# liaojing/videomorphing

Measured on AMD Instinct MI355X. Metric: Mpixel*iters/s (halfway optimizer, 1080p pair, 6-level pyramid, 500 iters/level), higher is better.
Workload: dtype f32

## Files before the change

### videomorphing_amd/csrc/vm_sweep_kernels.hip

```cpp
#include <algorithm>
#include <type_traits>
#include "vm_morph_common.h"

typedef __attribute__((address_space(1))) const uint32_t vm_g_cu32;
typedef __attribute__((address_space(1))) uint32_t vm_g_u32;
typedef __attribute__((address_space(1))) const unsigned long long vm_g_cu64;
typedef __attribute__((address_space(1))) unsigned long long vm_g_u64;
typedef __attribute__((address_space(1))) const float vm_g_cf32;

__device__ __forceinline__ int mad24(int a, int b, int c) { return __mul24(a, b) + c; }

namespace {

__device__ __forceinline__ int tile_cols(int w) { return (w + VM_PITCH_X - 1) / VM_PITCH_X; }
__device__ __forceinline__ int tile_rows(int h) { return (h + VM_PITCH_Y - 1) / VM_PITCH_Y; }
__device__ __forceinline__ int tile_ox(int t, int gx, int offx) { return (t % gx) * VM_PITCH_X + offx; }
__device__ __forceinline__ int tile_oy(int t, int gx, int offy) { return (t / gx) * VM_PITCH_Y + offy; }
__device__ __forceinline__ int phase_px(int ox, int slot, int pj) { return ox + (slot & 31) * 2 + pj; }
__device__ __forceinline__ int phase_py(int oy, int slot, int pi) { return oy + (slot >> 5) * 2 + pi; }
__device__ __forceinline__ void stage_imp(uint32_t *imp, const uint32_t *tables, int tid, int T) { for (int k = tid; k < 225; k += T) imp[k] = tables[VM_TAB_IMP + k]; }
__device__ __forceinline__ void stage_tps(float *tps, const uint32_t *tables, int tid, int T) { for (int k = tid; k < 625; k += T) tps[k] = __uint_as_float(tables[VM_TAB_TPS + k]); }
__device__ __forceinline__ float cell_count(int qy, int h, int qx, int w) { return (float)(window_count(qy, h) * window_count(qx, w)); }
__device__ __forceinline__ int window_row(int k) { return (k * 13) >> 6; }

struct TileLds {
    float2 mean[VM_NCELL], var[VM_NCELL], tpsb[VM_NCELL];
    float cross[VM_NCELL], value[VM_NCELL];
    float2 d_mean[256], d_var[256], d_step[256];
    float d_cross[256];
    int d_ok[256];
    int list[256];
    int wave_cnt[4];
    uint32_t cbits[8];
    float tps[625];
    uint32_t imp[225];
    uint32_t mask[6][16];
    uint32_t n_eval;
    uint32_t dirty[(VM_NCELL + 31) / 32];
};

struct SplitLds {
    float2 d_mean[256], d_var[256], d_step[256];
    float d_cross[256];
    int d_ok[256];
    int list[256];
    int wave_cnt[4];
    float tps[625];
    uint32_t imp[225];
    uint32_t mask[6][16];
    uint32_t n_eval;
};

struct PixelCtx {
    int px, py;
    int idx;
    float2 v, old_luma;
    float tps_axy, ui_axy;
    float2 tps_b, ui_b;
    float2 tref;
    float tmask;
};

__device__ __forceinline__ float temp_change(const PixelCtx &c, float dx, float dy)
{
    float v_temp = 0.0f;
    v_temp += fabsf(c.v.x + dx - c.tref.x) - fabsf(c.v.x - c.tref.x);
    v_temp += fabsf(c.v.y + dy - c.tref.y) - fabsf(c.v.y - c.tref.y);
    return v_temp;
}

template <bool TEMP>
__device__ __forceinline__ bool temp_on(const VmLevelView &L) { return TEMP && L.temp_mask != nullptr; }
#if VM_EXACT
#define VM_VARIANT_TEMPLATE
constexpr bool TEMP = true;
#else
// ... 647 lines not shown
    fi = __builtin_amdgcn_fmed3f(fi, -1.0f, (float)L.w);
    fj = __builtin_amdgcn_fmed3f(fj, -1.0f, (float)L.h);
    const int i = clamp0(L.w - 1, (int)fi + t.cx), j = clamp0(L.h - 1, (int)fj + t.cy);
    wgt = fmaf(t.wxs, a, t.wxo) * fmaf(t.wys, b, t.wyo);
    return (uint32_t)(t.imgoff + j * L.rs + i) << 2;
}
__device__ __forceinline__ void taps32_issue(const VmLevelView &L, const TapLane &t, const PixelCtx &c, float vx,
                                             float vy, float &texel, float &wgt)
{
    texel = *(vm_g_cf32 *)((const char *)L.img0 + taps32_addr(L, t, c, vx, vy, wgt));
}
struct TexelKeep {
    uint32_t off = 0xFFFFFFFFu;
    float texel = 0.0f;
};
__device__ __forceinline__ void taps32_issue(const VmLevelView &L, const TapLane &t, const PixelCtx &c, float vx,
                                             float vy, TexelKeep &keep, float &texel, float &wgt)
{
    const uint32_t off = taps32_addr(L, t, c, vx, vy, wgt);
    if (off != keep.off) {
        keep.texel = *(vm_g_cf32 *)((const char *)L.img0 + off);
        keep.off = off;
    }
    texel = keep.texel;
}
__device__ __forceinline__ void taps32_finish(const TapLane &t, float texel, float wgt, float &lx, float &ly)
{
    float r = texel * wgt;
    r += dpp_xor1(r);
    r += dpp_xor2(r);
    const float o = dpp_half_mirror(r);
    lx = t.odd ? o : r;
    ly = t.odd ? r : o;
}
template <int K>
__device__ __forceinline__ float ladder_take(float x)
{
    return __int_as_float(__builtin_amdgcn_ds_swizzle(__float_as_int(x), 0x07 | (K << 8)));
}
__device__ __forceinline__ void taps32(const VmLevelView &L, const TapLane &t, const PixelCtx &c, float vx, float vy,
                                       TexelKeep &keep, float &lx, float &ly)
{
    float texel, wgt;
    taps32_issue(L, t, c, vx, vy, keep, texel, wgt);
    taps32_finish(t, texel, wgt, lx, ly);
}
__device__ __forceinline__ void line_lumas(const VmLevelView &L, const TapLane &t, const PixelCtx &c, float gx, float gy,
                                           float tmin, TexelKeep &keep, float2 &luma)
{
    taps32(L, t, c, fmaf(gx, tmin, c.v.x), fmaf(gy, tmin, c.v.y), keep, luma.x, luma.y);
}

template <bool INTERIOR>
__device__ __forceinline__ float change32(const VmKParams &P, const Nb1 &nb, const PixelCtx &c, float lx, float ly)
{
    const float dmx = lx - c.old_luma.x, dmy = ly - c.old_luma.y;
    const float dvx = lx * lx - c.old_luma.x * c.old_luma.x;
    const float dvy = ly * ly - c.old_luma.y * c.old_luma.y;
    const float dcross = lx * ly - c.old_luma.x * c.old_luma.y;
    float acc;
    if (INTERIOR) {
        const float val = ssim_core(window_mean(nb.A, dmx, 0.04f), window_mean(nb.B, dmy, 0.04f), nb.VX + dvx, nb.VY + dvy,
                                    nb.X + dcross, 25.0f, P.ssim_clamp);
        acc = nb.N != 0.0f ? nb.VAL - val : 0.0f;
    } else {
        const bool valid = nb.N != 0.0f;
        const float n = valid ? nb.N : 25.0f;
        const float in = n == 25.0f ? 0.04f : __builtin_amdgcn_rcpf(n);
        const float val = ssim_core(window_mean(nb.A, dmx, in), window_mean(nb.B, dmy, in), nb.VX + dvx, nb.VY + dvy,
                                    nb.X + dcross, n, P.ssim_clamp);
        acc = valid ? nb.VAL - val : 0.0f;
    }
    return group_sum(acc, 32);
}

template <class Ring>
__device__ __forceinline__ float fover32(const VmLevelView &L, const Ring &ring, const PixelCtx &c, float gx, float gy,
                                         int sub)
{
    const int k = sub & 7, k1 = (k + 1) & 7;
    const float sgn = (sub & 8) ? 1.0f : -1.0f;
    const float vx = sgn * c.v.x, vy = sgn * c.v.y;
    float ex[2], ey[2];
#pragma unroll
    for (int e = 0; e < 2; ++e) {
        const int kk = e ? k1 : k;
        const int rx = ((0x06A4 >> (2 * kk)) & 3) - 1, ry = ((0x6A40 >> (2 * kk)) & 3) - 1;
        const int qx = c.px + rx, qy = c.py + ry;
        float ux = vx, uy = vy;
        const bool in = qx >= 0 && qx < L.w && qy >= 0 && qy < L.h;
        const float2 nv = ring(kk, in ? qy * L.rs + qx : c.idx);
        if (in) {
            ux = sgn * nv.x;
            uy = sgn * nv.y;
        }
        ex[e] = ux + (float)(c.px - rx);
        ey[e] = uy + (float)(c.py - ry);
    }
    float t_min = 10;
    fover_isec((float)c.px + vx, (float)c.py + vy, sgn * gx, sgn * gy, ex[0], ey[0], ex[1], ey[1], t_min);
    return group_min32(sub < 16 ? t_min : 10.0f);
}

template <bool INTERIOR, bool TEMP, class Ring>
__device__ __forceinline__ bool decide32(const VmLevelView &L, const VmKParams &P, const Nb1 &nb, const Ring &ring,
                                         const PixelCtx &c, int sub, float2 &step, float2 &luma,
                                         uint32_t &n_eval)
{
    n_eval += 4;
    const bool has_temp = temp_on<TEMP>(L);
    const float WT = has_temp ? P.w_temp * c.tmask * L.factor_d * L.inv_wh : 0.0f;
    const TapLane tl = tap_lane_make(L, sub);
    float lx, ly;
    float gx = 0, gy = 0;
    float g_tex[4], g_wgt[4];
#pragma unroll
    for (int k = 0; k < 4; ++k) {
        const float sgn = (k & 1) ? -1.0f : 1.0f;
        const float dx = k < 2 ? sgn * P.eps : 0.0f, dy = k < 2 ? 0.0f : sgn * P.eps;
        taps32_issue(L, tl, c, c.v.x + dx, c.v.y + dy, g_tex[k], g_wgt[k]);
    }
#pragma unroll
    for (int k = 0; k < 4; ++k) {
        const float sgn = (k & 1) ? -1.0f : 1.0f;
        const float dx = k < 2 ? sgn * P.eps : 0.0f, dy = k < 2 ? 0.0f : sgn * P.eps;
        taps32_finish(tl, g_tex[k], g_wgt[k], lx, ly);
// ... 38 lines not shown
    float b = cc * C, x = b * R + cc * C;
    float fb, fx;
    ELINE(b, fb);
    ELINE(x, fx);
#pragma unroll 1
    for (;;) {
        if (!(cc - a > P.eps))
            break;
        const bool lt = fx < fb;
        const float p = lt ? x : b, qv = lt ? cc : a;
        a = lt ? b : a;
        cc = lt ? cc : x;
        const float xn = p * R + qv * C;
        float f;
        ELINE(xn, f);
        const float ob = b, ofb = fb;
        b = lt ? x : xn;
        x = lt ? xn : ob;
        fb = lt ? fx : f;
        fx = lt ? f : ofb;
    }
#undef ELINE
    const float tmin = fx < fb ? x : b, fmin = fx < fb ? fx : fb;
    if (!(fmin < 0))
        return false;
    step = make_float2(gx * tmin, gy * tmin);
    line_lumas(L, tl, c, gx, gy, tmin, keep, luma);
    return true;
}


__device__ __forceinline__ float ladder_pick(bool hi, int oct, float l0, float h0, float l1, float h1, float l2, float h2,
                                             float l3, float h3)
{
    const float p0 = hi ? h0 : l0, p1 = hi ? h1 : l1, p2 = hi ? h2 : l2, p3 = hi ? h3 : l3;
    const float p01 = (oct & 1) ? p1 : p0, p23 = (oct & 1) ? p3 : p2;
    return (oct & 2) ? p23 : p01;
}
#define LADDER_FETCH(K_, BLX_, BLY_, PLX_, PLY_, LX_, LY_)  \
    {                                                       \
        if ((K_) == 0) {                                    \
            (LX_) = ladder_take<0>(BLX_);                   \
            (LY_) = ladder_take<0>(BLY_);                   \
        } else {                                            \
            (LX_) = (PLX_);                                 \
            (LY_) = (PLY_);                                 \
        }                                                   \
        if ((K_) != 3) {                                    \
            (PLX_) = ladder_take<((K_) + 1) & 3>(BLX_);     \
            (PLY_) = ladder_take<((K_) + 1) & 3>(BLY_);     \
        }                                                   \
    }
#define GOLDEN64_NO_TRACE(T_)
#define GOLDEN64_NO_BATCH(T_)
#define GOLDEN64_REGIME_ROUND(EVALB_, TRACE_, K_, CC_, EPS_, HI_, NEVAL_)                                              \
    {                                                                                                                  \
        const float xn = b * R, xn2 = xn * R;                                                                          \
        float f1, f2;                                                                                                  \
        EVALB_(K_, (HI_) ? xn2 : xn, f1, f2);                                                                          \
        TRACE_(xn)                                                                                                     \
              \
        const bool held = x > (EPS_) && !(fb < f1);                                                                    \
        if (held) {                           \
            TRACE_(xn2)                                                                                                \
        }                                                                                                              \
        (NEVAL_) += held ? 2 : 1;                                                                                      \
        (CC_) = held ? b : x;                                                                                          \
        x = held ? xn : b;                                                                                             \
        b = held ? xn2 : xn;                                                                                           \
        fx = held ? f1 : fb;                                                                                           \
        fb = held ? f2 : f1;                                                                                           \
    }
#define GOLDEN64(EVAL2_, BATCH_, EVALB_, TRACE_, CC_, EPS_, HI_, OCT_, NEVAL_, TMIN_, FMIN_)                           \
    {                                                                                                                  \
        const float R = 0.618033989f, C = 1.0f - R;                                                                    \
        float a = 0;                                                                                                   \
        float b = (CC_) * C, x = b * R + (CC_) * C;                                                                    \
        float fb, fx;                                                                                                  \
        {                     \
            const float q1 = b * R, q2 = q1 * R, q3 = q2 * R, q4 = q3 * R, q5 = q4 * R, q6 = q5 * R;                   \
            BATCH_(ladder_pick((HI_), (OCT_), b, x, q1, q2, q3, q4, q5, q6))                                           \
        }                                                                                                              \
        EVALB_(0, (HI_) ? x : b, fb, fx);                                                                              \
        TRACE_(b)                                                                                                      \
        TRACE_(x)                                                                                                      \
        (NEVAL_) += 2;                                                                                                 \
        _Pragma("unroll 1") for (;;) {                                          \
            if (!((CC_) > (EPS_) && !(fx < fb)))                                                                       \
                break;                                                                                                 \
            GOLDEN64_REGIME_ROUND(EVALB_, TRACE_, 1, CC_, EPS_, HI_, NEVAL_)                                           \
            if (!((CC_) > (EPS_) && !(fx < fb)))                                                                       \
                break;                                                                                                 \
            GOLDEN64_REGIME_ROUND(EVALB_, TRACE_, 2, CC_, EPS_, HI_, NEVAL_)                                           \
            if (!((CC_) > (EPS_) && !(fx < fb)))                                                                       \
                break;                                                                                                 \
            GOLDEN64_REGIME_ROUND(EVALB_, TRACE_, 3, CC_, EPS_, HI_, NEVAL_)                                           \
            if (!((CC_) > (EPS_) && !(fx < fb)))                                                                       \
                break;                                                                                                 \
            {                       \
                const float q1 = b * R, q2 = q1 * R, q3 = q2 * R, q4 = q3 * R, q5 = q4 * R, q6 = q5 * R, q7 = q6 * R,  \
                            q8 = q7 * R;                                                                               \
                BATCH_(ladder_pick((HI_), (OCT_), q1, q2, q3, q4, q5, q6, q7, q8))                                     \
            }                                                                                                          \
            GOLDEN64_REGIME_ROUND(EVALB_, TRACE_, 0, CC_, EPS_, HI_, NEVAL_)                                           \
        }                                                                                                              \
        _Pragma("unroll 1") for (;;)                                                                                   \
        {                                                                                                              \
            if (!((CC_) - a > (EPS_)))                                                                                 \
                break;                                                                                                 \
            const bool lt = fx < fb;                                                                                   \
                          \
            const float p = lt ? x : b, qv = lt ? (CC_) : a;                                                           \
            const float a1 = lt ? b : a, cc1 = lt ? (CC_) : x;                                                         \
            const float xn = p * R + qv * C;                                                                           \
            const float b1 = lt ? x : xn, x1 = lt ? xn : b;                                                            \
             \
               \
                      \
                                                                               \
            const bool G = lt;                                                                                         \
            const float p2 = G ? x1 : b1, q2 = G ? cc1 : a1;                                                           \
            const float xn2 = p2 * R + q2 * C;                                                                         \
            float f1, f2;                                                                                              \
            EVAL2_((HI_) ? xn2 : xn, f1, f2);                                                                          \
            TRACE_(xn)                                                                                                 \
            ++(NEVAL_);                                                                                                \
            {                                                                                                          \
                const float nfb = lt ? fx : f1, nfx = lt ? f1 : fb;                                                    \
                a = a1;                                                                                                \
                (CC_) = cc1;                                                                                           \
                b = b1;                                                                                                \
                x = x1;                                                                                                \
                fb = nfb;                                                                                              \
                fx = nfx;                                                                                              \
            }                                                                                                          \
            if ((CC_) - a > (EPS_) && (fx < fb) == G) {          \
                TRACE_(xn2)                                                                                            \
                const float ob = b, ofb = fb;                                                                          \
                a = G ? b : a;                                                                                         \
                (CC_) = G ? (CC_) : x;                                                                                 \
                b = G ? x : xn2;                                                                                       \
                x = G ? xn2 : ob;                                                                                      \
                fb = G ? fx : f2;                                                                                      \
                fx = G ? f2 : ofb;                                                                                     \
                ++(NEVAL_);                                                                                            \
            }                                                                                                          \
        }                                                                                                              \
        (TMIN_) = fx < fb ? x : b;                                                                                     \
        (FMIN_) = fx < fb ? fx : fb;                                                                                   \
    }

template <bool INTERIOR, bool LADDER, bool TEMP, class Ring>
__device__ __forceinline__ bool decide64(const VmLevelView &L, const VmKParams &P, const Nb1 &nb, const Ring &ring,
                                         const PixelCtx &c, int sub, bool hi, float2 &step, float2 &luma,
                                         uint32_t &n_eval)
{
    n_eval += 4;
    const bool has_temp = temp_on<TEMP>(L);
    const float WT = has_temp ? P.w_temp * c.tmask * L.factor_d * L.inv_wh : 0.0f;
    const TapLane tl = tap_lane_make(L, sub);
    float lx, ly;
    float gx = 0, gy = 0;
    {
        const float sgn = hi ? -1.0f : 1.0f;
        float g_tex[2], g_wgt[2];
#pragma unroll
        for (int r = 0; r < 2; ++r) {
            const float dx = r == 0 ? sgn * P.eps : 0.0f, dy = r == 0 ? 0.0f : sgn * P.eps;
            taps32_issue(L, tl, c, c.v.x + dx, c.v.y + dy, g_tex[r], g_wgt[r]);
        }
#pragma unroll
        for (int r = 0; r < 2; ++r) {
            const float dx = r == 0 ? sgn * P.eps : 0.0f, dy = r == 0 ? 0.0f : sgn * P.eps;
            taps32_finish(tl, g_tex[r], g_wgt[r], lx, ly);
            const float change = change32<INTERIOR>(P, nb, c, lx, ly);
            const float dd = dx * dx + dy * dy;
            const float v_tps = fmaf(c.tps_axy, dd, fmaf(c.tps_b.x, dx, c.tps_b.y * dy));
            const float v_ui = fmaf(c.ui_axy, dd, fmaf(c.ui_b.x, dx, c.ui_b.y * dy));
            float e = (P.w_ui * v_ui + P.w_ssim * change) * L.inv_wh + P.w_tps * v_tps;
            if (has_temp)
                e = fmaf(WT, temp_change(c, dx, dy), e);
            e *= sgn;
            float e_lo, e_hi;
            halves(e, e_lo, e_hi);
            if (r == 0) {
                gx += e_lo;
                gx += e_hi;
            } else {
                gy += e_lo;
                gy += e_hi;
            }
        }
    }
    gx = -gx;
    gy = -gy;
    const float ng = fsqrt(gx * gx + gy * gy);
    if (ng == 0)
        return false;
    gx = fdiv(gx, ng);
    gy = fdiv(gy, ng);
    float cc = fmaxf(fover32(L, ring, c, gx, gy, sub) - P.eps, 0.0f);
    const float gg = gx * gx + gy * gy;
    const float WS = P.w_ssim * L.inv_wh, WU = P.w_ui * L.inv_wh;
    const float Q2 = (WU * c.ui_axy + P.w_tps * c.tps_axy) * gg;
    const float Q1 = WU * (c.ui_b.x * gx + c.ui_b.y * gy) + P.w_tps * (c.tps_b.x * gx + c.tps_b.y * gy);
    const float T0 = fabsf(c.v.x - c.tref.x) + fabsf(c.v.y - c.tref.y);
    TexelKeep keep;
#define ELINE2(T_, FLO_, FHI_)                                                         \
    {                                                                                  \
        const float nvx_ = fmaf(gx, (T_), c.v.x), nvy_ = fmaf(gy, (T_), c.v.y);        \
        taps32(L, tl, c, nvx_, nvy_, keep, lx, ly);                                    \
        float f_ = fmaf(WS, change32<INTERIOR>(P, nb, c, lx, ly), (T_) * fmaf(Q2, (T_), Q1)); \
        if (has_temp)                                                                  \
            f_ = fmaf(WT, (fabsf(nvx_ - c.tref.x) + fabsf(nvy_ - c.tref.y)) - T0, f_); \
        halves(f_, (FLO_), (FHI_));                                                    \
    }
    float blx, bly;
    float plx, ply;
#define LADDER2(T_)                                                                             \
    if (LADDER)                                                                                 \
        taps32(L, tl, c, fmaf(gx, (T_), c.v.x), fmaf(gy, (T_), c.v.y), keep, blx, bly);
#define ELINE2B(K_, T_, FLO_, FHI_)                                                    \
    {                                                                                  \
        const float nvx_ = fmaf(gx, (T_), c.v.x), nvy_ = fmaf(gy, (T_), c.v.y);        \
        if (LADDER)                                                                    \
            LADDER_FETCH(K_, blx, bly, plx, ply, lx, ly)                               \
        else                                                                           \
            taps32(L, tl, c, nvx_, nvy_, keep, lx, ly);                                \
        float f_ = fmaf(WS, change32<INTERIOR>(P, nb, c, lx, ly), (T_) * fmaf(Q2, (T_), Q1)); \
        if (has_temp)                                                                  \
            f_ = fmaf(WT, (fabsf(nvx_ - c.tref.x) + fabsf(nvy_ - c.tref.y)) - T0, f_); \
        halves(f_, (FLO_), (FHI_));                                                    \
    }
    float tmin, fmin;
    GOLDEN64(ELINE2, LADDER2, ELINE2B, GOLDEN64_NO_TRACE, cc, P.eps, hi, sub >> 3, n_eval, tmin, fmin)
#undef ELINE2
#undef ELINE2B
#undef LADDER2
    if (!(fmin < 0))
        return false;
    step = make_float2(gx * tmin, gy * tmin);
    line_lumas(L, tl, c, gx, gy, tmin, keep, luma);
    return true;
}
#endif

template <bool TEMP = true>
__device__ __forceinline__ void ctx_load(PixelCtx &c, const VmLevelView &L, const float *s_tps, int px, int py)
{
    c.px = px;
    c.py = py;
    c.idx = py * L.rs + px;
    c.v = L.v[c.idx];
    c.old_luma = L.luma[c.idx];
    c.ui_axy = L.ui_axy[c.idx];
    c.ui_b = L.ui_b[c.idx];
    c.tps_axy = s_tps[(border_class(py, L.h) * 5 + border_class(px, L.w)) * 25 + 12] / 2;
    c.tref = make_float2(0, 0);
    c.tmask = 0.0f;
    if (temp_on<TEMP>(L)) {
        c.tref = L.temp_ref[c.idx];
        c.tmask = L.temp_mask[c.idx];
    }
}

__device__ __forceinline__ bool is_interior(const VmLevelView &L, int px, int py)
{
    return px >= 4 && px < L.w - 4 && py >= 4 && py < L.h - 4;
}

struct MaskGeom {
    int bx0, by0, nbx, nby;
};
__device__ __forceinline__ MaskGeom mask_geom(int w, int h, int ox, int oy)
{
    MaskGeom g;
    g.bx0 = ox / 5 - 1;
    g.by0 = oy / 5 - 1;
    const int bx1 = min(ox + VM_TILE_W - 1, w - 1) / 5 + 1;
    const int by1 = min(oy + VM_TILE_H - 1, h - 1) / 5 + 1;
    g.nbx = bx1 - g.bx0 + 1;
    g.nby = by1 - g.by0 + 1;
    return g;
}
__device__ __forceinline__ MaskGeom mask_geom(const VmLevelView &L, int ox, int oy) { return mask_geom(L.w, L.h, ox, oy); }

__device__ __forceinline__ bool mask_hit(const uint32_t (*mask)[16], const uint32_t *imp, const MaskGeom &g,
                                         int px, int py)
{
    const int oxb = px % 5, oyb = py % 5;
// ... 800 lines not shown
        for (int pj = 0; pj < 2; ++pj) {
            const int vx = V.vx, vy = V.vy;
            const int vpi = pi ^ ((oy - vy) & 1), vpj = pj ^ ((ox - vx) & 1);
            int *const ph_cnt = Q.ph_cnt[pj];
            uint32_t *const ph_cand = Q.ph_cand[pj], *const ph_commit = Q.ph_commit[pj];
            bool cand = false, hit = false;
            uint32_t *mword = nullptr;
            uint32_t mbit = 0;
            if (tid < 256) {
                const int px = vx + (tid & 31) * 2 + vpj, py = vy + (tid >> 5) * 2 + vpi;
                if (px >= ox && px <= rx1 && py >= oy && py <= ry1 && mask_hit(S.mask, S.imp, V.g, px, py)) {
                    hit = true;
                    cand = !pixel_locked(L, P.bcond, px, py);
                    mword = &S.mask[py / 5 - V.g.by0][px / 5 - V.g.bx0];
                    mbit = 1u << ((px % 5) + (py % 5) * 5);
                }
                const unsigned long long bc = __ballot(cand), bh = __ballot(hit);
                if ((tid & 63) == 0) {
                    ph_cand[(tid >> 6) * 2] = (uint32_t)bc;
                    ph_cand[(tid >> 6) * 2 + 1] = (uint32_t)(bc >> 32);
                    ph_cnt[tid >> 6] = __popcll(bc) | (bh ? 1 << 16 : 0);
                    ph_commit[(tid >> 6) * 2] = 0;
                    ph_commit[(tid >> 6) * 2 + 1] = 0;
                }
            }
            __syncthreads();
            const int w0 = ph_cnt[0], w1 = ph_cnt[1], w2 = ph_cnt[2], w3 = ph_cnt[3];
            if (!((w0 | w1 | w2 | w3) >> 16))
                continue;
            const int n_act = (w0 & 0xFFFF) + (w1 & 0xFFFF) + (w2 & 0xFFFF) + (w3 & 0xFFFF);
            if (hit && !cand)
                atomicAnd(mword, ~mbit);
            if (n_act > 0) {
                st_cand += n_act;
                const bool wide = n_act * 64 <= T;
                for (int base = 0; base < n_act; base += wide ? T / 64 : T / 32) {
                    const int li = base + (wide ? tid >> 6 : tid >> 5), sub = tid & 31;
                    const bool writer = wide ? (tid & 63) == 0 : sub == 0;
                    const int slot = sv_kth_slot(ph_cand, min(li, n_act - 1));
                    const int tx = slot & 31, ty = slot >> 5;
                    const int px = vx + tx * 2 + vpj, py = vy + ty * 2 + vpi;
                    const bool wave_interior = __all(li >= n_act || is_interior(L, px, py));
                    if (li < n_act) {
                        LdsSrc src{&S, (ty * 2 + vpi) * VM_HALO_W + (tx * 2 + vpj)};
                        const int pc = src.hc + 2 * VM_HALO_W + 2;
                        PixelCtx c;
                        c.px = px;
                        c.py = py;
                        c.idx = py * L.rs + px;
                        c.v = X.v[pc];
                        c.old_luma = X.luma[pc];
                        c.ui_axy = X.uiaxy[pc];
                        c.ui_b = X.uib[pc];
                        c.tps_axy = S.tps[(border_class(py, L.h) * 5 + border_class(px, L.w)) * 25 + 12] / 2;
                        c.tref = make_float2(0, 0);
                        c.tmask = 0.0f;
                        if (temp_on<TEMP>(L)) {
                            c.tref = L.temp_ref[c.idx];
                            c.tmask = L.temp_mask[c.idx];
                        }
                        c.tps_b = S.tpsb[pc];
                        const RingLds ring{X.v, pc};
                        float2 step, luma;
                        Nb1 nb;
                        bool ok;
                        uint32_t n_eval = 0;
                        if (wave_interior) {
                            nb1_load<true>(nb, L, src, c, sub);
                            ok = wide ? decide64<true, true, TEMP>(L, P, nb, ring, c, sub, (tid & 32) != 0, step, luma, n_eval)
                                      : decide32<true, TEMP>(L, P, nb, ring, c, sub, step, luma, n_eval);
                        } else {
                            nb1_load<false>(nb, L, src, c, sub);
                            ok = wide ? decide64<false, true, TEMP>(L, P, nb, ring, c, sub, (tid & 32) != 0, step, luma, n_eval)
                                      : decide32<false, TEMP>(L, P, nb, ring, c, sub, step, luma, n_eval);
                        }
                        if (writer) {
                            atomicAdd(&S.n_eval, n_eval);
                            uint32_t *const mw = &S.mask[py / 5 - V.g.by0][px / 5 - V.g.bx0];
                            const uint32_t mb = 1u << ((px % 5) + (py % 5) * 5);
                            if (ok) {
                                S.d_step[slot] = step;
                                S.d_mean[slot] = commit_dmean(luma, c.old_luma);
                                S.d_var[slot] = commit_dvar(luma, c.old_luma);
                                S.d_cross[slot] = commit_dcross(luma.x, luma.y, c.old_luma.x, c.old_luma.y);
                                X.luma[pc] = luma;
                                X.uib[pc] = commit_ui_b(c.ui_b, c.ui_axy, step);
                                X.v[pc] = commit_v(c.v, step);
                                atomicOr(&X.dirty[pc >> 5], 1u << (pc & 31));
                                atomicOr(&ph_commit[ty], 1u << tx);
                                atomicOr(mw, mb);
                                if (res && (res > 1 || !sv_safe(L, V, px, py)))
                                    Q.unsafe = 1u;
                            } else
                                atomicAnd(mw, ~mb);
                        }
                    }
                }
            }
            __syncthreads();

            uint32_t cb[8];
            int ncommit = 0, ty0 = 8, ty1 = -1;
#pragma unroll
            for (int k = 0; k < 8; ++k) {
                cb[k] = ph_commit[k];
                ncommit += __popc(cb[k]);
                if (cb[k]) {
// ... 662 lines not shown
                                          int qy, float2 &m, float2 &q, float &cr, float2 &tb, int order)
{
#if !VM_EXACT
    (void)order;
#endif
    const bool touched = hits != 0;
#pragma unroll
    for (int half = 0; half < 2; ++half) {
        if (!__any(hits != 0))
            break;
        float4 ra[5], rb[5];
        int bidx[5];
#pragma unroll
        for (int k = 0; k < 5; ++k) {
            if (half == 1 && k == 4) {
                bidx[k] = -1;
                continue;
            }
#if VM_EXACT
            int b = -1;
            if (hits) {
                if (!(order & 2)) {
                    b = (order & 1) ? 31 - __clz(hits) : __ffs(hits) - 1;
                } else {
                    const uint32_t ht = transpose5(hits);
                    const int bt = (order & 1) ? 31 - __clz(ht) : __ffs(ht) - 1;
                    b = (bt % 5) * 5 + bt / 5;
                }
                hits &= ~(1u << b);
            }
#else
            const int b = hits ? __ffs(hits) - 1 : -1;
            hits &= hits - 1;
#endif
            bidx[k] = b;
            const int bb = max(b, 0);
            const int dy = window_row(bb), dx = bb - dy * 5;
            const int rsafe = b >= 0 ? (qy + dy - 2) * L.rs + (qx + dx - 2) : qy * L.rs + qx;
            ra[k] = rec_load<COH>(r_a + rsafe);
            rb[k] = rec_load<COH>(r_b + rsafe);
        }
#pragma unroll
        for (int k = 0; k < 5; ++k) {
            const int b = bidx[k];
            if (b < 0)
                continue;
            const int dy = window_row(b), dx = b - dy * 5;
            const int x = qx + dx - 2, y = qy + dy - 2;
            m.x += ra[k].x;
            m.y += ra[k].y;
            q.x += ra[k].z;
            q.y += ra[k].w;
            cr += rb[k].x;
            const float kk = s_tps[(border_class(y, L.h) * 5 + border_class(x, L.w)) * 25 + (4 - dy) * 5 + (4 - dx)];
            tb.x += rb[k].y * kk;
            tb.y += rb[k].z * kk;
        }
    }
    return touched;
}

template <int T, bool TEMP = true>
__global__ __launch_bounds__(T) __attribute__((amdgpu_waves_per_eu(T / 128))) void SUF(k_step)(const VmLevelView *__restrict__ views, int cap, VmKParams P,
                                                   const uint32_t *__restrict__ tables, int offx, int offy, int pi,
                                                   int pj, int parts, uint32_t epoch, uint32_t pe, int srcbuf,
                                                   int n_fold, uint32_t *__restrict__ flags,
                                                   uint32_t *__restrict__ stats, int iter_idx, int fixed_work,
                                                   uint32_t *__restrict__ slots_cur, const uint32_t *__restrict__ slots_prev,
                                                   int prev_iter_idx, int nslot)
{
    __shared__ StepLds S;
    const int tid = threadIdx.x;
    const VmLevelView L = views[blockIdx.z];
    flags += (size_t)blockIdx.z * cap;
    stats += (size_t)blockIdx.z * cap * VM_STAT_WORDS;
    const bool s1 = srcbuf == 1, d1 = srcbuf == 0;
    const float2 *s_mean = s1 ? L.mean2 : L.mean, *s_var = s1 ? L.var2 : L.var, *s_tpsb = s1 ? L.tps_b2 : L.tps_b;
    const float *s_cross = s1 ? L.cross2 : L.cross, *s_value = s1 ? L.value2 : L.value;
    const uint32_t *s_imp = s1 ? L.impmask2 : L.impmask;
    float2 *d_mean = d1 ? L.mean2 : L.mean, *d_var = d1 ? L.var2 : L.var, *d_tpsb = d1 ? L.tps_b2 : L.tps_b;
    float *d_cross = d1 ? L.cross2 : L.cross, *d_value = d1 ? L.value2 : L.value;
    uint32_t *d_imp = d1 ? L.impmask2 : L.impmask;
    const bool in_place = srcbuf == 2;
    const bool r1 = pe & 1u, w1 = epoch & 1u;
    const uint32_t *r_tag = r1 ? L.rec_tag2 : L.rec_tag;
    const float4 *r_a = r1 ? L.rec_a2 : L.rec_a, *r_b = r1 ? L.rec_b2 : L.rec_b;
    uint32_t *w_tag = w1 ? L.rec_tag2 : L.rec_tag;
    float4 *w_a = w1 ? L.rec_a2 : L.rec_a, *w_b = w1 ? L.rec_b2 : L.rec_b;
    const uint32_t want = (pe << 2) | 1u;

    stage_tps(S.tps, tables, tid, T);
    if (tid < VM_STEP_BH * 4)
        S.bits[tid >> 2][tid & 3] = 0;

    if ((int)blockIdx.x < n_fold) {
        const int nfx = (L.w + 63) / 64;
        const int x0 = ((int)blockIdx.x % nfx) * 64, y0 = ((int)blockIdx.x / nfx) * 16;
        const int bx0 = x0 - 2, by0 = y0 - 2;
        constexpr int NTF = (68 * 20 + T - 1) / T, NCF = 1024 / T;
        uint32_t tg[NTF];
#pragma unroll
        for (int e = 0; e < NTF; ++e) {
            const int k = tid + e * T;
            const int x = bx0 + k % 68, y = by0 + k / 68;
            tg[e] = (k < 68 * 20 && x >= 0 && x < L.w && y >= 0 && y < L.h) ? r_tag[y * L.rs + x] : 0u;
        }
        float2 cm[NCF], cq[NCF], ctb[NCF];
// ... 543 lines not shown
            a_ok[r] = ph > 0 && sub < 25 && x >= ox && x < tx1 && y >= oy && y < ty1;
            a_tag[r] = o_rtag + ((uint32_t)(a_ok[r] ? mad24(y, L.rs, x) : pidx) << 2);
        }
        bool b_ok;
        uint32_t b_tag;
        {
            const int x = 5 * wbx + sub % 5, y = 5 * wby + sub / 5;
            b_ok = ph > 0 && has_word && sub < 25 && x >= ox && x < tx1 && y >= oy && y < ty1;
            b_tag = o_rtag + ((uint32_t)(b_ok ? mad24(y, L.rs, x) : pidx) << 2);
        }
        const int sx0 = -4 + ((ppj ^ pj) & 1), sy0 = -4 + ((ppi ^ pi) & 1);
        bool c_ok;
        uint32_t c_tag, c_rec;
        {
            const int dx = sx0 + 2 * (sub % 5), dy = sy0 + 2 * (sub / 5);
            const int x = px + dx, y = py + dy;
            c_ok = ph > 0 && sub < 25 && dx <= 4 && dy <= 4 && x >= ox && x < tx1 && y >= oy && y < ty1;
            const uint32_t ri = (uint32_t)(c_ok ? mad24(y, L.rs, x) : pidx);
            c_tag = o_rtag + (ri << 2);
            c_rec = (hi ? o_rb : o_ra) + (ri << 4);
        }
        const int phx = 2 + 2 * tx + pj, phy = 2 + 2 * ty + pi;
        const int ohx0 = tx == 0 ? 0 : phx, ohx1 = tx == 31 ? VM_HALO_W - 1 : phx + 1;
        const int ohy0 = ty == 0 ? 0 : phy, ohy1 = ty == 7 ? VM_HALO_H - 1 : phy + 1;
        const int wi_ = window_row(sub), wj_ = sub - wi_ * 5;
        int chx, chy;
        if (sub < 25) {
            chx = phx + wj_ - 2;
            chy = phy + wi_ - 2;
        } else {
            const int xcol = (tx == 0 && pj == 1) ? 0 : ((tx == 31 && pj == 0) ? VM_HALO_W - 1 : -1);
            const int xrow = (ty == 0 && pi == 1) ? 0 : ((ty == 7 && pi == 0) ? VM_HALO_H - 1 : -1);
            const int ncol = xcol >= 0 ? ohy1 - ohy0 + 1 : 0;
            const int e = (sub - 25) + (hi ? 7 : 0);
            chx = chy = -1;
            if (e < ncol) {
                chx = xcol;
                chy = ohy0 + e;
            } else if (xrow >= 0) {
                int k = ohx0 + (e - ncol);
                if (xcol >= 0 && xcol == ohx0)
                    ++k;
                if (k <= ohx1 && k != xcol) {
                    chx = k;
                    chy = xrow;
                }
            }
        }
        const int qx = ox - 2 + chx, qy = oy - 2 + chy;
        const bool cell_ok = chx >= 0 && qx >= 0 && qx < L.w && qy >= 0 && qy < L.h;
        const bool okc = cell_ok && sub < 25;
        const uint32_t gi = (uint32_t)(cell_ok ? mad24(qy, L.rs, qx) : pidx);
        const uint32_t g4 = gi << 2, g8 = gi << 3;
        const float tps_axy = S.tps[(border_class(spy, L.h) * 5 + border_class(spx, L.w)) * 25 + 12] / 2;
        __builtin_amdgcn_sched_barrier(0);
        uint32_t mword[2], mcanon[2], mtag[2];
#pragma unroll
        for (int r = 0; r < 2; ++r) {
            mword[r] = ldo<uint32_t>(sbase, os_imp + a_word[r]);
            mcanon[r] = ldo<uint32_t>(sb, o_imp + a_word[r]);
            mtag[r] = ldo<uint32_t>(wb, a_tag[r]);
        }
        uint32_t otag = ldo<uint32_t>(wb, b_tag);
        uint32_t ctag = ldo<uint32_t>(wb, c_tag);
        const float4 crec = ldo<float4>(wb, c_rec);
        float2 m = ldo<float2>(sbase, os_mean + g8), q = ldo<float2>(sbase, os_var + g8), tb = ldo<float2>(sbase, os_tpsb + g8);
        float cr = ldo<float>(sbase, os_cross + g4), val = ldo<float>(sbase, os_value + g4);
        c.tref = make_float2(0, 0);
        c.tmask = 0.0f;
        if (temp_on<TEMP>(L)) {
            c.tref = L.temp_ref[pidx];
            c.tmask = L.temp_mask[pidx];
        }
        __builtin_amdgcn_sched_barrier(0);
        c.tps_axy = tps_axy;
#pragma unroll
        for (int r = 0; r < 2; ++r) {
            if (!a_owned[r])
                mword[r] = mcanon[r];
            if (!a_ok[r])
                mtag[r] = 0;
        }
        if (!b_ok)
            otag = 0;
        if (!c_ok)
            ctag = 0;

        if (ph > 0) {
            const uint32_t setb = (uint32_t)__ballot(!hi && otag == want);
            const uint32_t clrb = (uint32_t)__ballot(!hi && otag == ((pe << 2) | 2u));
            if (has_word && lane == 0)
                sto<uint32_t>(dbase, od_imp + w4, (oword | setb) & ~clrb, wt);
        }
        bool touched = false;
        if (ph > 0) {
            const uint32_t cset = (uint32_t)__ballot(!hi && ctag == want);
            if (cset) {
                if (sub < 25 && ctag == want)
                    S.rec[wave][(sub / 5 + 1) * 7 + sub % 5 + 1][hi ? 1 : 0] = crec;
                __builtin_amdgcn_wave_barrier();
                const int cdx = chx - phx, cdy = chy - phy;
                const int i0 = (cdx - 2 - sx0 + 1) >> 1, j0 = (cdy - 2 - sy0 + 1) >> 1;
                const int e0x = sx0 + 2 * i0 - cdx, e0y = sy0 + 2 * j0 - cdy;
                const float4 *rbase = &S.rec[wave][(j0 + 1) * 7 + i0 + 1][0];
                uint32_t win[3];
                int bcx[3], bcy[3];
#pragma unroll
                for (int t = 0; t < 3; ++t) {
                    const int jj = j0 + t;
                    const uint32_t row = (jj >= 0 && jj <= 4) ? (cset >> (5 * jj)) & 31u : 0u;
                    win[t] = cell_ok ? ((row << 1) >> (i0 + 1)) & 7u : 0u;
                    if (e0y + 2 * t > 2)
                        win[t] = 0;
                    bcx[t] = border_class(px + sx0 + 2 * (i0 + t), L.w);
                    bcy[t] = border_class(py + sy0 + 2 * jj, L.h);
                }
                if (e0x + 4 > 2) {
                    win[0] &= 3u;
                    win[1] &= 3u;
                    win[2] &= 3u;
                }
                float4 ra[9], rb[9];
                float kk[9];
#pragma unroll
                for (int k = 0; k < 9; ++k) {
                    const int a = k % 3, t = k / 3;
                    ra[k] = rbase[(t * 7 + a) * 2];
                    rb[k] = rbase[(t * 7 + a) * 2 + 1];
                    const bool u = (win[t] >> a) & 1u;
                    kk[k] = S.tps[u ? (bcy[t] * 5 + bcx[a]) * 25 + (2 - e0y - 2 * t) * 5 + (2 - e0x - 2 * a) : 0];
                }
#pragma unroll
                for (int k0 = 0; k0 < 9; ++k0) {
#if VM_EXACT
                    const int kr = (P.commit_order & 1) ? 8 - k0 : k0;
                    const int k = (P.commit_order & 2) ? (kr % 3) * 3 + kr / 3 : kr;
#else
                    const int k = k0;
#endif
                    if ((win[k / 3] >> (k % 3)) & 1u) {
                        touched = true;
                        m.x += ra[k].x;
                        m.y += ra[k].y;
                        q.x += ra[k].z;
                        q.y += ra[k].w;
                        cr += rb[k].x;
                        tb.x += rb[k].y * kk[k];
                        tb.y += rb[k].z * kk[k];
                    }
                }
                __builtin_amdgcn_wave_barrier();
            }
            if (touched) {
                const float counter = cell_count(qy, L.h, qx, L.w);
                val = ssim_value(m.x, m.y, q.x, q.y, cr, counter, P.ssim_clamp);
            }
            const bool owned = cell_ok && chx >= ohx0 && chx <= ohx1 && chy >= ohy0 && chy <= ohy1 && (sub >= 25 || !hi);
            if (owned) {
                sto<float2>(dbase, od_mean + g8, m, wt);
                sto<float2>(dbase, od_var + g8, q, wt);
                sto<float>(dbase, od_cross + g4, cr, wt);
                sto<float2>(dbase, od_tpsb + g8, tb, wt);
                sto<float>(dbase, od_value + g4, val, wt);
            }
        }
        if (closing)
            break;

// ... 73 lines not shown
            }
        }
    }
    if (lane == 0) {
        atomicAdd(&S.n_cand, my_cand);
        atomicAdd(&S.n_commit, my_commit);
        atomicAdd(&S.n_eval, my_eval);
    }
    __syncthreads();
    if (tid == 0) {
        if (S.n_commit)
            flags[iter_idx] = 1u;
        *my_slot = make_uint4(S.n_cand, S.n_commit, S.n_eval, part == 0 ? 1u : 0u);
        if (b == 0)
            clock_probe(stats0 + (size_t)iter_idx * VM_STAT_WORDS, true);
    }
}

__global__ __launch_bounds__(64) void SUF(k_pass_tail)(uint32_t *__restrict__ stats, const uint32_t *__restrict__ slots_prev,
                                                        int prev_iter_idx, int nslot_prev, int ntiles, int ngroups, int cap, int spread)
{
    pass_sum_slots(stats, slots_prev, prev_iter_idx, nslot_prev, ntiles, ngroups, cap, (int)threadIdx.x, spread != 0);
}

__global__ void SUF(k_next_iter)(int *iter_dev, int set, int value)
{
    if (threadIdx.x == 0 && blockIdx.x == 0)
        *iter_dev = set ? value : *iter_dev + value;
}

#if !VM_EXACT
__global__ __launch_bounds__(64) void SUF(k_dbg_golden)(const float *__restrict__ in, float eps, uint32_t *__restrict__ out)
{
    const int k = (int)blockIdx.x;
    const bool hi = (threadIdx.x & 32) != 0;
    float cc = in[4 * k];
    const float A = in[4 * k + 1], t0 = in[4 * k + 2], B = in[4 * k + 3];
    uint32_t *o = out + (size_t)k * VM_DBG_GOLDEN_WORDS;
    uint32_t n_eval = 0;
    int n_pt = 0;
#define EGOLDEN(T_, FLO_, FHI_)                     \
    {                                               \
        const float d_ = (T_) - t0;                 \
        const float f_ = (A * d_) * d_ + B;         \
        halves(f_, (FLO_), (FHI_));                 \
    }
#define TGOLDEN(T_)                                             \
    {                                                           \
        if (threadIdx.x == 0 && n_pt < VM_DBG_GOLDEN_WORDS - 3) \
            o[3 + n_pt] = __float_as_uint(T_);                  \
        ++n_pt;                                                 \
    }
#define EGOLDENB(K_, T_, FLO_, FHI_) EGOLDEN(T_, FLO_, FHI_)
    float tmin, fmin;
    GOLDEN64(EGOLDEN, GOLDEN64_NO_BATCH, EGOLDENB, TGOLDEN, cc, eps, hi, 0, n_eval, tmin, fmin)
#undef EGOLDENB
#undef EGOLDEN
#undef TGOLDEN
    if (threadIdx.x == 0) {
        o[0] = __float_as_uint(tmin);
        o[1] = __float_as_uint(fmin);
        o[2] = n_eval;
    }
}

__global__ __launch_bounds__(64) void SUF(k_dbg_ladder)(const float *__restrict__ img, int w, int h, const float *__restrict__ in,
                                                        float eps, uint32_t *__restrict__ out)
{
    const int k = (int)blockIdx.x;
    const bool hi = (threadIdx.x & 32) != 0;
    const int sub = (int)threadIdx.x & 31;
    const float *q = in + 8 * k;
    VmLevelView L = {};
    L.w = w;
    L.h = h;
    L.rs = w;
    L.img0 = img;
    L.img1 = img + w * h;
    PixelCtx c = {};
    c.px = (int)q[0];
    c.py = (int)q[1];
    c.v = make_float2(q[2], q[3]);
    const float gx = q[4], gy = q[5];
    float cc = q[6];
    uint32_t *o = out + (size_t)k * VM_DBG_LADDER_WORDS;
    const TapLane tl = tap_lane_make(L, sub);
    TexelKeep keep, keep_one;
    float blx, bly, plx = 0.0f, ply = 0.0f;
    uint32_t n_eval = 0;
    int n_pt = 0;
#define RLADDER(T_, LX_, LY_)                                                                                   \
    {                                                                                                           \
        float ox_, oy_;                                                                                         \
        taps32(L, tl, c, fmaf(gx, (T_), c.v.x), fmaf(gy, (T_), c.v.y), keep_one, ox_, oy_);                     \
        const int s_ = n_pt + (hi ? 1 : 0);                                                                     \
        if (sub == 0 && s_ < VM_DBG_LADDER_POINTS) {                                                            \
            o[1 + 5 * s_] = __float_as_uint(T_);                                                                \
            o[2 + 5 * s_] = __float_as_uint(LX_);                                                               \
            o[3 + 5 * s_] = __float_as_uint(LY_);                                                               \
            o[4 + 5 * s_] = __float_as_uint(ox_);                                                               \
            o[5 + 5 * s_] = __float_as_uint(oy_);                                                               \
        }                                                                                                       \
        n_pt += 2;                                                                                              \
    }
#define BLADDER(T_) taps32(L, tl, c, fmaf(gx, (T_), c.v.x), fmaf(gy, (T_), c.v.y), keep, blx, bly);
#define ELADDERB(K_, T_, FLO_, FHI_)                     \
    {                                                    \
        float lx_, ly_;                                  \
        LADDER_FETCH(K_, blx, bly, plx, ply, lx_, ly_)   \
        RLADDER(T_, lx_, ly_)                            \
        halves((T_), (FLO_), (FHI_));                    \
    }
#define ELADDER(T_, FLO_, FHI_)                                                              \
    {                                                                                        \
        float lx_, ly_;                                                                      \
        taps32(L, tl, c, fmaf(gx, (T_), c.v.x), fmaf(gy, (T_), c.v.y), keep, lx_, ly_);      \
        RLADDER(T_, lx_, ly_)                                                                \
        halves((T_), (FLO_), (FHI_));                                                        \
    }
    float tmin, fmin;
    GOLDEN64(ELADDER, BLADDER, ELADDERB, GOLDEN64_NO_TRACE, cc, eps, hi, sub >> 3, n_eval, tmin, fmin)
#undef ELADDER
#undef ELADDERB
#undef BLADDER
#undef RLADDER
    (void)tmin;
    (void)fmin;
    if (threadIdx.x == 0)
        o[0] = (uint32_t)n_pt;
}
#endif

}

#if VM_EXACT
#define VM_VARIANT_LAUNCH(TEMPORAL_, KERNEL_, ...) hipLaunchKernelGGL(KERNEL_(true), __VA_ARGS__)
#else
#define VM_VARIANT_LAUNCH(TEMPORAL_, KERNEL_, ...)           \
    do {                                                     \
        if (TEMPORAL_)                                       \
            hipLaunchKernelGGL(KERNEL_(true), __VA_ARGS__);  \
        else                                                 \
            hipLaunchKernelGGL(KERNEL_(false), __VA_ARGS__); \
    } while (0)
#endif
void SUF(vm_launch_optimize)(const VmLevelView *views, int nbatch, int cap, int w, int h, const VmKParams &P,
                             const uint32_t *tables, int offx, int offy, uint32_t *flags, uint32_t *stats,
                             int iter_idx, int fixed_work, int threads, const int *iter_dev, int dense,
                             uint32_t *tile_list, int temporal, hipStream_t s)
{
    dim3 b(threads), g((w + VM_PITCH_X - 1) / VM_PITCH_X, (h + VM_PITCH_Y - 1) / VM_PITCH_Y, nbatch);
    (void)temporal;
#define K_TILE_(TEMP_) (SUF(k_optimize)<true, VM_SMAX, VM_MIN_FANOUT, true, TEMP_>)
#if !VM_EXACT
#define K_LISTED_(TEMP_) (SUF(k_optimize_listed)<TEMP_>)
#define K_LEAN_(TEMP_) (SUF(k_optimize)<false, VM_SMAX, VM_MIN_FANOUT, true, TEMP_>)
#define K_TILE128_(TEMP_) (SUF(k_optimize)<true, 7, 4, true, TEMP_>)
#define K_TILE_NOINT_(TEMP_) (SUF(k_optimize)<true, VM_SMAX, VM_MIN_FANOUT, false, TEMP_>)
    if (!dense && tile_list) {
        const int nwords = ((w + 4) / 5 + 2) * ((h + 4) / 5 + 2), tiles = (int)(g.x * g.y);
        hipLaunchKernelGGL(SUF(k_tile_scan), dim3(std::min((nwords + 255) / 256, 32), 1, nbatch), dim3(256), 0, s, views, cap, offx,
                           offy, flags, iter_idx, fixed_work, iter_dev, tile_list, tiles);
        VM_VARIANT_LAUNCH(temporal, K_LISTED_, dim3(std::min(tiles * nbatch, VM_TILE_LIST_GRID)), b, 0, s, views, cap, P, tables,
                          offx, offy, flags, stats, iter_idx, iter_dev, tile_list, tiles, nbatch);
        return;
    }
    if (!dense) {
        VM_VARIANT_LAUNCH(temporal, K_LEAN_, g, b, 0, s, views, cap, P, tables, offx, offy, flags, stats,
                          iter_idx, fixed_work, iter_dev);
        return;
    }
    if (dense == 2) {
        VM_VARIANT_LAUNCH(temporal, K_TILE128_, g, b, 0, s, views, cap, P, tables, offx, offy, flags, stats,
                          iter_idx, fixed_work, iter_dev);
        return;
// ... 148 lines not shown
```

Baseline: 2060.

## Interleave SSIM change evaluation with cross-lane reductions in golden line search

Splits change32 into a per-lane part and a reduction. In the ladder path of the golden-section search, the SSIM change for the next ladder point is now computed while the DPP reduction of the current point runs, with sched barriers fencing the interleave. The two gradient probes are also finished and reduced as a pair, and border_class is replaced by a branchless min/max form. The aim is to hide the latency of the serial DPP/swizzle reduction chains behind independent ALU work. In exchange, the hand-placed scheduling constraints could limit the compiler and raise register pressure.

After: 2085 (median of 6 runs). 1.01x the previous value.

```diff
diff --git a/videomorphing_amd/csrc/vm_sweep_kernels.hip b/videomorphing_amd/csrc/vm_sweep_kernels.hip
--- a/videomorphing_amd/csrc/vm_sweep_kernels.hip
+++ b/videomorphing_amd/csrc/vm_sweep_kernels.hip
@@ -22,6 +22,21 @@
 __device__ __forceinline__ void stage_tps(float *tps, const uint32_t *tables, int tid, int T) { for (int k = tid; k < 625; k += T) tps[k] = __uint_as_float(tables[VM_TAB_TPS + k]); }
 __device__ __forceinline__ float cell_count(int qy, int h, int qx, int w) { return (float)(window_count(qy, h) * window_count(qx, w)); }
 __device__ __forceinline__ int window_row(int k) { return (k * 13) >> 6; }
+
+#ifndef VM_CHAIN_BESIDE
+#define VM_CHAIN_BESIDE 1
+#endif
+#ifndef VM_CHAIN_SELECTS
+#define VM_CHAIN_SELECTS 1
+#endif
+__device__ __forceinline__ int border_class_in(int p, int dim)
+{
+#if VM_CHAIN_SELECTS
+    return min(p, min(max(p - dim + 5, 2), 4));
+#else
+    return border_class(p, dim);
+#endif
+}
 
 struct TileLds {
     float2 mean[VM_NCELL], var[VM_NCELL], tpsb[VM_NCELL];
@@ -775,7 +790,7 @@
 }
 
 template <bool INTERIOR>
-__device__ __forceinline__ float change32(const VmKParams &P, const Nb1 &nb, const PixelCtx &c, float lx, float ly)
+__device__ __forceinline__ float change32_lane(const VmKParams &P, const Nb1 &nb, const PixelCtx &c, float lx, float ly)
 {
     const float dmx = lx - c.old_luma.x, dmy = ly - c.old_luma.y;
     const float dvx = lx * lx - c.old_luma.x * c.old_luma.x;
@@ -794,7 +809,92 @@
                                     nb.X + dcross, n, P.ssim_clamp);
         acc = valid ? nb.VAL - val : 0.0f;
     }
-    return group_sum(acc, 32);
+    return acc;
+}
+template <bool INTERIOR>
+__device__ __forceinline__ float change32(const VmKParams &P, const Nb1 &nb, const PixelCtx &c, float lx, float ly)
+{
+    return group_sum(change32_lane<INTERIOR>(P, nb, c, lx, ly), 32);
+}
+#define VM_SCHED_FENCE() __builtin_amdgcn_sched_barrier(0)
+__device__ __forceinline__ void group_sum32_pair(float &x, float &y)
+{
+    VM_SCHED_FENCE();
+    x += dpp_xor1(x);
+    y += dpp_xor1(y);
+    VM_SCHED_FENCE();
+    x += dpp_xor2(x);
+    y += dpp_xor2(y);
+    VM_SCHED_FENCE();
+    x += dpp_half_mirror(x);
+    y += dpp_half_mirror(y);
+    VM_SCHED_FENCE();
+    x += dpp_mirror(x);
+    y += dpp_mirror(y);
+    VM_SCHED_FENCE();
+    const float sx = swz_xor16(x), sy = swz_xor16(y);
+    x += sx;
+    y += sy;
+}
+template <bool INTERIOR>
+__device__ __forceinline__ float change32_lane_beside_sum(const VmKParams &P, const Nb1 &nb, const PixelCtx &c, float nlx,
+                                                          float nly, float &sum)
+{
+    const bool valid = nb.N != 0.0f;
+    const float n = INTERIOR ? 25.0f : (valid ? nb.N : 25.0f);
+    const float in = INTERIOR ? 0.04f : (n == 25.0f ? 0.04f : __builtin_amdgcn_rcpf(n));
+    const float nc2 = n * 58.5225f, nc3 = n * 29.26125f;
+    VM_SCHED_FENCE();
+    const float dmx = nlx - c.old_luma.x, dmy = nly - c.old_luma.y;
+    const float xx = nlx * nlx, yy = nly * nly, xy = nlx * nly;
+    VM_SCHED_FENCE();
+    sum += dpp_xor1(sum);
+    VM_SCHED_FENCE();
+    const float dvx = xx - c.old_luma.x * c.old_luma.x;
+    const float dvy = yy - c.old_luma.y * c.old_luma.y;
+    const float dcross = xy - c.old_luma.x * c.old_luma.y;
+    const float a = window_mean(nb.A, dmx, in), b = window_mean(nb.B, dmy, in);
+    VM_SCHED_FENCE();
+    sum += dpp_xor2(sum);
+    VM_SCHED_FENCE();
+    const float sx2 = nb.VX + dvx, sy2 = nb.VY + dvy, sxy = nb.X + dcross;
+    const float na = n * a, nbb = n * b;
+    const float vx = fmaxf(fmaf(-na, a, sx2), 0.0f);
+    const float vy = fmaxf(fmaf(-nbb, b, sy2), 0.0f);
+    VM_SCHED_FENCE();
+    sum += dpp_half_mirror(sum);
+    VM_SCHED_FENCE();
+    const float cov = fmaf(-na, b, sxy);
+    const float ss = __builtin_amdgcn_sqrtf(vx * vy);
+    VM_SCHED_FENCE();
+    sum += dpp_mirror(sum);
+    const float other = swz_xor16(sum);
+    VM_SCHED_FENCE();
+    const float num = fmaf(2.0f, ss, nc2) * (fabsf(cov) + nc3);
+    const float den = ((vx + vy) + nc2) * (ss + nc3);
+    const float val = fmaxf(fminf(num * __builtin_amdgcn_rcpf(den), 1.0f), P.ssim_clamp);
+    float acc = valid ? nb.VAL - val : 0.0f;
+    asm volatile("" : "+v"(acc));
+    VM_SCHED_FENCE();
+    sum += other;
+    return acc;
+}
+__device__ __forceinline__ void taps32_finish_pair(const TapLane &t, float texel0, float wgt0, float texel1, float wgt1,
+                                                   float &lx0, float &ly0, float &lx1, float &ly1)
+{
+    float r0 = texel0 * wgt0, r1 = texel1 * wgt1;
+    VM_SCHED_FENCE();
+    r0 += dpp_xor1(r0);
+    r1 += dpp_xor1(r1);
+    VM_SCHED_FENCE();
+    r0 += dpp_xor2(r0);
+    r1 += dpp_xor2(r1);
+    VM_SCHED_FENCE();
+    const float o0 = dpp_half_mirror(r0), o1 = dpp_half_mirror(r1);
+    lx0 = t.odd ? o0 : r0;
+    ly0 = t.odd ? r0 : o0;
+    lx1 = t.odd ? o1 : r1;
+    ly1 = t.odd ? r1 : o1;
 }
 
 template <class Ring>
@@ -939,12 +1039,18 @@
         }                                                   \
     }
 #define GOLDEN64_NO_TRACE(T_)
+#define GOLDEN64_ROUND_PLAIN(EVALB_, K_, B_, R_, HI_, XN_, XN2_, FLO_, FHI_) \
+    {                                                                        \
+        (XN_) = (B_) * (R_);                                                 \
+        (XN2_) = (XN_) * (R_);                                               \
+        EVALB_(K_, (HI_) ? (XN2_) : (XN_), FLO_, FHI_);                      \
+    }
 #define GOLDEN64_NO_BATCH(T_)
-#define GOLDEN64_REGIME_ROUND(EVALB_, TRACE_, K_, CC_, EPS_, HI_, NEVAL_)                                              \
+#define GOLDEN64_REGIME_ROUND(EVALR_, TRACE_, K_, CC_, EPS_, HI_, NEVAL_)                                              \
     {                                                                                                                  \
-        const float xn = b * R, xn2 = xn * R;                                                                          \
+        float xn, xn2;                    \
         float f1, f2;                                                                                                  \
-        EVALB_(K_, (HI_) ? xn2 : xn, f1, f2);                                                                          \
+        EVALR_(K_, b, R, (HI_), xn, xn2, f1, f2);                                                                      \
         TRACE_(xn)                                                                                                     \
               \
         const bool held = x > (EPS_) && !(fb < f1);                                                                    \
@@ -958,7 +1064,7 @@
         fx = held ? f1 : fb;                                                                                           \
         fb = held ? f2 : f1;                                                                                           \
     }
-#define GOLDEN64(EVAL2_, BATCH_, EVALB_, TRACE_, CC_, EPS_, HI_, OCT_, NEVAL_, TMIN_, FMIN_)                           \
+#define GOLDEN64(EVAL2_, BATCH_, EVALB_, EVALR_, TRACE_, CC_, EPS_, HI_, OCT_, NEVAL_, TMIN_, FMIN_)                   \
     {                                                                                                                  \
         const float R = 0.618033989f, C = 1.0f - R;                                                                    \
         float a = 0;                                                                                                   \
@@ -975,13 +1081,13 @@
         _Pragma("unroll 1") for (;;) {                                          \
             if (!((CC_) > (EPS_) && !(fx < fb)))                                                                       \
                 break;                                                                                                 \
-            GOLDEN64_REGIME_ROUND(EVALB_, TRACE_, 1, CC_, EPS_, HI_, NEVAL_)                                           \
+            GOLDEN64_REGIME_ROUND(EVALR_, TRACE_, 1, CC_, EPS_, HI_, NEVAL_)                                           \
             if (!((CC_) > (EPS_) && !(fx < fb)))                                                                       \
                 break;                                                                                                 \
-            GOLDEN64_REGIME_ROUND(EVALB_, TRACE_, 2, CC_, EPS_, HI_, NEVAL_)                                           \
+            GOLDEN64_REGIME_ROUND(EVALR_, TRACE_, 2, CC_, EPS_, HI_, NEVAL_)                                           \
             if (!((CC_) > (EPS_) && !(fx < fb)))                                                                       \
                 break;                                                                                                 \
-            GOLDEN64_REGIME_ROUND(EVALB_, TRACE_, 3, CC_, EPS_, HI_, NEVAL_)                                           \
+            GOLDEN64_REGIME_ROUND(EVALR_, TRACE_, 3, CC_, EPS_, HI_, NEVAL_)                                           \
             if (!((CC_) > (EPS_) && !(fx < fb)))                                                                       \
                 break;                                                                                                 \
             {                       \
@@ -989,7 +1095,7 @@
                             q8 = q7 * R;                                                                               \
                 BATCH_(ladder_pick((HI_), (OCT_), q1, q2, q3, q4, q5, q6, q7, q8))                                     \
             }                                                                                                          \
-            GOLDEN64_REGIME_ROUND(EVALB_, TRACE_, 0, CC_, EPS_, HI_, NEVAL_)                                           \
+            GOLDEN64_REGIME_ROUND(EVALR_, TRACE_, 0, CC_, EPS_, HI_, NEVAL_)                                           \
         }                                                                                                              \
         _Pragma("unroll 1") for (;;)                                                                                   \
         {                                                                                                              \
@@ -1037,7 +1143,7 @@
         (FMIN_) = fx < fb ? fx : fb;                                                                                   \
     }
 
-template <bool INTERIOR, bool LADDER, bool TEMP, class Ring>
+template <bool INTERIOR, bool LADDER, bool TEMP, bool BESIDE = LADDER && VM_CHAIN_BESIDE, class Ring>
 __device__ __forceinline__ bool decide64(const VmLevelView &L, const VmKParams &P, const Nb1 &nb, const Ring &ring,
                                          const PixelCtx &c, int sub, bool hi, float2 &step, float2 &luma,
                                          uint32_t &n_eval)
@@ -1056,11 +1162,16 @@
             const float dx = r == 0 ? sgn * P.eps : 0.0f, dy = r == 0 ? 0.0f : sgn * P.eps;
             taps32_issue(L, tl, c, c.v.x + dx, c.v.y + dy, g_tex[r], g_wgt[r]);
         }
+        float g_lx[2], g_ly[2], g_chg[2];
+        taps32_finish_pair(tl, g_tex[0], g_wgt[0], g_tex[1], g_wgt[1], g_lx[0], g_ly[0], g_lx[1], g_ly[1]);
+#pragma unroll
+        for (int r = 0; r < 2; ++r)
+            g_chg[r] = change32_lane<INTERIOR>(P, nb, c, g_lx[r], g_ly[r]);
+        group_sum32_pair(g_chg[0], g_chg[1]);
 #pragma unroll
         for (int r = 0; r < 2; ++r) {
             const float dx = r == 0 ? sgn * P.eps : 0.0f, dy = r == 0 ? 0.0f : sgn * P.eps;
-            taps32_finish(tl, g_tex[r], g_wgt[r], lx, ly);
-            const float change = change32<INTERIOR>(P, nb, c, lx, ly);
+            const float change = g_chg[r];
             const float dd = dx * dx + dy * dy;
             const float v_tps = fmaf(c.tps_axy, dd, fmaf(c.tps_b.x, dx, c.tps_b.y * dy));
             const float v_ui = fmaf(c.ui_axy, dd, fmaf(c.ui_b.x, dx, c.ui_b.y * dy));
@@ -1108,7 +1219,9 @@
     if (LADDER)                                                                                 \
         taps32(L, tl, c, fmaf(gx, (T_), c.v.x), fmaf(gy, (T_), c.v.y), keep, blx, bly);
 #define ELINE2B(K_, T_, FLO_, FHI_)                                                    \
-    {                                                                                  \
+    if (LADDER && BESIDE)                                                              \
+        ELINE2P(K_, T_, FLO_, FHI_)                                                    \
+    else {                                                                             \
         const float nvx_ = fmaf(gx, (T_), c.v.x), nvy_ = fmaf(gy, (T_), c.v.y);        \
         if (LADDER)                                                                    \
             LADDER_FETCH(K_, blx, bly, plx, ply, lx, ly)                               \
@@ -1119,10 +1232,49 @@
             f_ = fmaf(WT, (fabsf(nvx_ - c.tref.x) + fabsf(nvy_ - c.tref.y)) - T0, f_); \
         halves(f_, (FLO_), (FHI_));                                                    \
     }
+    float sn = 0.0f;
+#define ELINE2P(K_, T_, FLO_, FHI_)                                                    \
+    {                                                                                  \
+        float s_, nlx_, nly_;                                                          \
+        if ((K_) == 0) {                                                               \
+            lx = ladder_take<0>(blx);                                                  \
+            ly = ladder_take<0>(bly);                                                  \
+            nlx_ = ladder_take<1>(blx);                                                \
+            nly_ = ladder_take<1>(bly);                                                \
+            plx = ladder_take<2>(blx);                                                 \
+            ply = ladder_take<2>(bly);                                                 \
+            s_ = change32_lane<INTERIOR>(P, nb, c, lx, ly);                            \
+        } else {                                                                       \
+            s_ = sn;                                                                   \
+            nlx_ = plx;                                                                \
+            nly_ = ply;                                                                \
+            if ((K_) == 1) {                                                           \
+                plx = ladder_take<3>(blx);                                             \
+                ply = ladder_take<3>(bly);                                             \
+            }                                                                          \
+        }                                                                              \
+        const float tq_ = (T_) * fmaf(Q2, (T_), Q1);                                   \
+        float tt_ = 0.0f;                                                              \
+        if (has_temp) {                                                                \
+            const float nvx_ = fmaf(gx, (T_), c.v.x), nvy_ = fmaf(gy, (T_), c.v.y);    \
+            tt_ = (fabsf(nvx_ - c.tref.x) + fabsf(nvy_ - c.tref.y)) - T0;              \
+        }                                                                              \
+        if ((K_) != 3)                                                                 \
+            sn = change32_lane_beside_sum<INTERIOR>(P, nb, c, nlx_, nly_, s_);         \
+        else                                                                           \
+            s_ = group_sum(s_, 32);                                                    \
+        float f_ = fmaf(WS, s_, tq_);                                                  \
+        if (has_temp)                                                                  \
+            f_ = fmaf(WT, tt_, f_);                                                    \
+        halves(f_, (FLO_), (FHI_));                                                    \
+    }
+#define ELINE2R(K_, B_, R_, HI_, XN_, XN2_, FLO_, FHI_) GOLDEN64_ROUND_PLAIN(ELINE2B, K_, B_, R_, HI_, XN_, XN2_, FLO_, FHI_)
     float tmin, fmin;
-    GOLDEN64(ELINE2, LADDER2, ELINE2B, GOLDEN64_NO_TRACE, cc, P.eps, hi, sub >> 3, n_eval, tmin, fmin)
+    GOLDEN64(ELINE2, LADDER2, ELINE2B, ELINE2R, GOLDEN64_NO_TRACE, cc, P.eps, hi, sub >> 3, n_eval, tmin, fmin)
 #undef ELINE2
+#undef ELINE2R
 #undef ELINE2B
+#undef ELINE2P
 #undef LADDER2
     if (!(fmin < 0))
         return false;
@@ -2029,7 +2181,7 @@
                         c.old_luma = X.luma[pc];
                         c.ui_axy = X.uiaxy[pc];
                         c.ui_b = X.uib[pc];
-                        c.tps_axy = S.tps[(border_class(py, L.h) * 5 + border_class(px, L.w)) * 25 + 12] / 2;
+                        c.tps_axy = S.tps[(border_class_in(py, L.h) * 5 + border_class_in(px, L.w)) * 25 + 12] / 2;
                         c.tref = make_float2(0, 0);
                         c.tmask = 0.0f;
                         if (temp_on<TEMP>(L)) {
@@ -2798,7 +2950,7 @@
             q.x += ra[k].z;
             q.y += ra[k].w;
             cr += rb[k].x;
-            const float kk = s_tps[(border_class(y, L.h) * 5 + border_class(x, L.w)) * 25 + (4 - dy) * 5 + (4 - dx)];
+            const float kk = s_tps[(border_class_in(y, L.h) * 5 + border_class_in(x, L.w)) * 25 + (4 - dy) * 5 + (4 - dx)];
             tb.x += rb[k].y * kk;
             tb.y += rb[k].z * kk;
         }
@@ -3448,7 +3600,7 @@
         const bool okc = cell_ok && sub < 25;
         const uint32_t gi = (uint32_t)(cell_ok ? mad24(qy, L.rs, qx) : pidx);
         const uint32_t g4 = gi << 2, g8 = gi << 3;
-        const float tps_axy = S.tps[(border_class(spy, L.h) * 5 + border_class(spx, L.w)) * 25 + 12] / 2;
+        const float tps_axy = S.tps[(border_class_in(spy, L.h) * 5 + border_class_in(spx, L.w)) * 25 + 12] / 2;
         __builtin_amdgcn_sched_barrier(0);
         uint32_t mword[2], mcanon[2], mtag[2];
 #pragma unroll
@@ -3508,8 +3660,8 @@
                     win[t] = cell_ok ? ((row << 1) >> (i0 + 1)) & 7u : 0u;
                     if (e0y + 2 * t > 2)
                         win[t] = 0;
-                    bcx[t] = border_class(px + sx0 + 2 * (i0 + t), L.w);
-                    bcy[t] = border_class(py + sy0 + 2 * jj, L.h);
+                    bcx[t] = border_class_in(px + sx0 + 2 * (i0 + t), L.w);
+                    bcy[t] = border_class_in(py + sy0 + 2 * jj, L.h);
                 }
                 if (e0x + 4 > 2) {
                     win[0] &= 3u;
@@ -3689,8 +3841,10 @@
         ++n_pt;                                                 \
     }
 #define EGOLDENB(K_, T_, FLO_, FHI_) EGOLDEN(T_, FLO_, FHI_)
+#define EGOLDENR(K_, B_, R_, HI_, XN_, XN2_, FLO_, FHI_) GOLDEN64_ROUND_PLAIN(EGOLDENB, K_, B_, R_, HI_, XN_, XN2_, FLO_, FHI_)
     float tmin, fmin;
-    GOLDEN64(EGOLDEN, GOLDEN64_NO_BATCH, EGOLDENB, TGOLDEN, cc, eps, hi, 0, n_eval, tmin, fmin)
+    GOLDEN64(EGOLDEN, GOLDEN64_NO_BATCH, EGOLDENB, EGOLDENR, TGOLDEN, cc, eps, hi, 0, n_eval, tmin, fmin)
+#undef EGOLDENR
 #undef EGOLDENB
 #undef EGOLDEN
 #undef TGOLDEN
@@ -3748,6 +3902,7 @@
         RLADDER(T_, lx_, ly_)                            \
         halves((T_), (FLO_), (FHI_));                    \
     }
+#define ELADDERR(K_, B_, R_, HI_, XN_, XN2_, FLO_, FHI_) GOLDEN64_ROUND_PLAIN(ELADDERB, K_, B_, R_, HI_, XN_, XN2_, FLO_, FHI_)
 #define ELADDER(T_, FLO_, FHI_)                                                              \
     {                                                                                        \
         float lx_, ly_;                                                                      \
@@ -3756,8 +3911,9 @@
         halves((T_), (FLO_), (FHI_));                                                        \
     }
     float tmin, fmin;
-    GOLDEN64(ELADDER, BLADDER, ELADDERB, GOLDEN64_NO_TRACE, cc, eps, hi, sub >> 3, n_eval, tmin, fmin)
+    GOLDEN64(ELADDER, BLADDER, ELADDERB, ELADDERR, GOLDEN64_NO_TRACE, cc, eps, hi, sub >> 3, n_eval, tmin, fmin)
 #undef ELADDER
+#undef ELADDERR
 #undef ELADDERB
 #undef BLADDER
 #undef RLADDER
```
